# guzba/zippy

Hardware: NVIDIA H100
Metric: compress_level1_gzip_input_throughput (higher is better)
Workload: dtype u8

## Files before the change

zippy_b200/csrc/zb_deflate.cu:

```cuda
#include "zb_device.cuh"
#include "zb_kernels.h"
#include "zb_huff_warp.cuh"

#define LZ_THREADS (ZB_WARPS_PER_CHUNK * 32)
#define LZ_HASH_BITS 11
#define LZ_TABLE_ENTRIES (1 << LZ_HASH_BITS)
#define LZ_PRESEED 2048
#ifndef ZB_LZ1_RESOLVE_WINNER
#define ZB_LZ1_RESOLVE_WINNER 0
#endif
#define LZ_LANE_CAP 32

#define LZ_PIECE_BYTES ZB_REC_PIECE_BYTES
#define LZ_PHASES (ZB_SUB_BYTES / LZ_PIECE_BYTES)
#define LZ_PHASE_BYTES (ZB_CHUNK_BYTES / LZ_PHASES)
#define LZ_PHASE_HIST 1024
#define LZ_BATCH_LPW 2
#define LZ_BATCH_WINDOWS (32 / LZ_BATCH_LPW)
static_assert(LZ_PIECE_BYTES * ZB_WARPS_PER_CHUNK == LZ_PHASE_BYTES, "one piece per warp and phase");
static_assert(LZ_PIECE_BYTES / ZB_WINDOW % LZ_BATCH_WINDOWS == 0, "a batch of windows never straddles two pieces");

#define LZ_SM_DATA 0
#define LZ_SM_DATA_BYTES (LZ_PHASE_BYTES + LZ_PHASE_HIST + 64 + 384)
#define LZ_SM_TABLE (LZ_SM_DATA + LZ_SM_DATA_BYTES)
#define LZ_SM_TABLE_BYTES (ZB_WARPS_PER_CHUNK * LZ_TABLE_ENTRIES * 2)
#define LZ_SM_HIST (LZ_SM_TABLE + LZ_SM_TABLE_BYTES)
#define LZ_SM_HIST_BYTES (ZB_WARPS_PER_CHUNK * ZB_HIST_WORDS * 4)
#define LZ_SM_RING (LZ_SM_HIST + LZ_SM_HIST_BYTES)
#define LZ_SM_RING_BYTES (ZB_WARPS_PER_CHUNK * LZ_BATCH_WINDOWS * ZB_MATCH_SLOTS * 4)
#define LZ_SM_LMUL (LZ_SM_RING + LZ_SM_RING_BYTES)
#define LZ_LMUL_PIECE 33
#define LZ_LMUL_PQ 49
#define LZ_SM_LMUL_BYTES (56 * 4)
#define LZ_SM_PART (LZ_SM_LMUL + LZ_SM_LMUL_BYTES)
#define LZ_SM_PART_BYTES (ZB_WARPS_PER_CHUNK * 24)
#define LZ_SM_BAR (LZ_SM_PART + LZ_SM_PART_BYTES)
#define LZ_SM_TOTAL (LZ_SM_BAR + 16)
static_assert(LZ_TABLE_ENTRIES * 2 >= 4096, "a warp's table region must hold the CRC step table");
static_assert(3 * (LZ_SM_TOTAL + 1024) <= 233472, "three CTAs per SM");
static_assert(LZ_SM_PART % 8 == 0 && LZ_SM_TABLE % 16 == 0, "alignment");

__device__ __forceinline__ uint32_t lz_hash(uint32_t v) { return (v * 0x9E3779B1u) >> (32 - LZ_HASH_BITS); }
__device__ __forceinline__ uint32_t shl_clamp(uint32_t x, uint32_t n) {
  uint32_t r;
  asm("shl.b32 %0, %1, %2;" : "=r"(r) : "r"(x), "r"(n));
  return r;
}
__device__ __forceinline__ uint32_t low_mask(uint32_t n) { return shl_clamp(1u, n) - 1u; }

__device__ __forceinline__ uint32_t lz_final_rec(uint32_t mlen, uint32_t dist, int &lc, int &dc) {
  uint32_t le, de;
  lc = (int)zb_len_code_bf(mlen, le);
  dc = (int)zb_dist_code_bf(dist, de);
  return (uint32_t)lc | (le << 5) | ((uint32_t)dc << 10) | (de << 15);
}


__device__ __forceinline__ void lz_select(const uint8_t *data, uint32_t off0, uint32_t wb, uint32_t b1, uint32_t cur,
                                          uint32_t nvalid, uint32_t &m, uint32_t dist, uint32_t *ring_slot,
                                          uint32_t &sel, uint32_t &ism, uint32_t &endw) {
  const int lane = zb_lane();
  const uint32_t mm = __ballot_sync(ZB_FULL, m != 0);
  endw = 0;
  ism = 0;
  if (mm) {
    const uint32_t lbit = 1u << lane;
    const uint32_t endp = (uint32_t)lane + m;
    const uint32_t rest = shl_clamp(1u, endp) ? (mm >> endp) : 0u;
    uint32_t nc = rest ? endp + (uint32_t)(__ffs((int)rest) - 1) : 32u;
    uint32_t vis = 1u << (cur + (uint32_t)(__ffs((int)(mm >> cur)) - 1));
#pragma unroll
    for (int r = 0; r < 3; r++) {
      vis |= __reduce_or_sync(ZB_FULL, (vis & lbit) ? shl_clamp(1u, nc) : 0u);
      const uint32_t t = __shfl_sync(ZB_FULL, nc, (int)(nc & 31u));
      nc = nc < 32u ? t : 32u;
    }
    ism = vis;
    const int lastm = 31 - __clz((int)ism);
    const uint32_t cov = (ism & lbit) ? (low_mask(endp) & ~low_mask((uint32_t)lane)) : 0u;
    const uint32_t covered = __reduce_or_sync(ZB_FULL, cov);
    uint32_t mlast = __shfl_sync(ZB_FULL, m, lastm);
    if (mlast >= LZ_LANE_CAP) {
      const uint32_t md = __shfl_sync(ZB_FULL, dist, lastm);
      const uint32_t pos = wb + (uint32_t)lastm;
      const uint32_t off = off0 + pos + LZ_LANE_CAP + 8u * (uint32_t)lane;
      uint32_t x0 = zb_ld32_unaligned(data, off) ^ zb_ld32_unaligned(data, off - md);
      uint32_t x1 = zb_ld32_unaligned(data, off + 4) ^ zb_ld32_unaligned(data, off + 4 - md);
      uint32_t nm = x0 ? ((uint32_t)(__ffs((int)x0) - 1) >> 3) : 4u + (x1 ? ((uint32_t)(__ffs((int)x1) - 1) >> 3) : 4u);
      uint32_t stop = __ballot_sync(ZB_FULL, nm < 8u);
      if (stop) {
        int first = __ffs((int)stop) - 1;
        mlast = LZ_LANE_CAP + 8u * (uint32_t)first + __shfl_sync(ZB_FULL, nm, first);
      } else {
        mlast = LZ_LANE_CAP + 256u;
      }
      mlast = min(mlast, min((uint32_t)ZB_MAX_MATCH, b1 - pos));
      if (lane == lastm) m = mlast;
    }
    sel = ism | (~covered & ~low_mask(cur) & low_mask(nvalid));
    endw = (uint32_t)lastm + mlast;
    if (ism & lbit) {
      uint32_t rank = (uint32_t)__popc(ism & (lbit - 1u));
      ring_slot[rank] = (m - 3u) | ((dist - 1u) << 9);
    }
  } else {
    sel = low_mask(nvalid) & ~low_mask(cur);
  }
}

template <int LPW, bool LITS>
__device__ __forceinline__ void lz_batch_pass(const uint8_t *wdata, bool active, uint32_t ksel, uint32_t kism,
                                              const uint32_t *ring_win, uint32_t *whist, uint2 *gmask_w,
                                              uint32_t *grecs_piece, uint32_t &rec_base) {
  constexpr int NW = 32 / LPW;
  const uint32_t part = (uint32_t)zb_lane() / NW, wi = (uint32_t)zb_lane() % NW;
  if (active && part == 0) *gmask_w = make_uint2(ksel, kism);
  const uint32_t im = active ? kism : 0u;
  const uint32_t pm = (0xffffffffu >> (32 - 32 / LPW)) << (part * (32 / LPW));
  uint32_t s = (LITS && active) ? (ksel & ~kism & pm) : 0u;
  while (s) {
    const uint32_t bit = (uint32_t)(__ffs((int)s) - 1);
    s &= s - 1;
    const uint32_t sy = wdata[bit];
    atomicAdd(&whist[sy >> 1], 1u << ((sy & 1u) * 16u));
  }
  const uint32_t nmatch = (uint32_t)__popc(im);
  uint32_t incl = nmatch;
#pragma unroll
  for (int o = 1; o < NW; o <<= 1) {
    const uint32_t t = __shfl_up_sync(ZB_FULL, incl, o, NW);
    if (wi >= (uint32_t)o) incl += t;
  }
  uint32_t *grecs_w = grecs_piece + rec_base + incl - nmatch;
  rec_base += __shfl_sync(ZB_FULL, incl, NW - 1);
  for (uint32_t k = part; k < nmatch; k += LPW) {
    const uint32_t raw = ring_win[k];
    int lc, dc;
    const uint32_t fin = lz_final_rec((raw & 511u) + 3u, (raw >> 9) + 1u, lc, dc);
    grecs_w[k] = fin;
    const uint32_t s1 = 257u + (uint32_t)lc, s2 = (uint32_t)ZB_NUM_LITLEN + (uint32_t)dc;
    atomicAdd(&whist[s1 >> 1], 1u << ((s1 & 1u) * 16u));
    atomicAdd(&whist[s2 >> 1], 1u << ((s2 & 1u) * 16u));
  }
}

#ifndef ZB_LZ1_STAGE_CLOCKS
#define ZB_LZ1_STAGE_CLOCKS 0
#endif
enum { LZS_WAIT, LZS_CHECKSUM, LZS_SEED, LZS_PROBE, LZS_EXTEND, LZS_SELECT, LZS_BATCH, LZS_BARRIER, LZS_N };
#if ZB_LZ1_STAGE_CLOCKS
__device__ unsigned long long zb_lz1_stage_clk[LZS_N];
#define LZ_CLK_DECL                          \
  unsigned long long clk_acc[LZS_N] = {};    \
  long long clk_t = clock64();
#define LZ_CLK(s)                            \
  if (MODE == 1) {                           \
    const long long clk_n = clock64();       \
    clk_acc[s] += (unsigned long long)(clk_n - clk_t); \
    clk_t = clk_n;                           \
  }
#define LZ_CLK_PUBLISH()                                                                           \
  if (MODE == 1 && lane == 0) {                                                                    \
    _Pragma("unroll") for (int s_ = 0; s_ < LZS_N; s_++) atomicAdd(&zb_lz1_stage_clk[s_], clk_acc[s_]); \
  }
extern "C" int zb200_lz1_stage_clocks(unsigned long long *out) {
  unsigned long long zero[LZS_N] = {};
  if (cudaMemcpyFromSymbol(out, zb_lz1_stage_clk, sizeof(zero)) != cudaSuccess) return -1;
  return cudaMemcpyToSymbol(zb_lz1_stage_clk, zero, sizeof(zero)) == cudaSuccess ? 0 : -1;
}
#else
#define LZ_CLK_DECL
#define LZ_CLK(s)
#define LZ_CLK_PUBLISH()
#endif

template <int MODE, int CK>
__global__ void __launch_bounds__(LZ_THREADS, 3)
    k_lz(const uint8_t *__restrict__ src, const ZbChunkDesc *__restrict__ desc, uint2 *__restrict__ masks,
         uint32_t *__restrict__ recs, uint16_t *__restrict__ hist, ZbChunkCheck *__restrict__ chk,
         const ZbCrcTables *__restrict__ tabs, uint32_t max_dist) {
  extern __shared__ __align__(128) uint8_t smem[];
  uint8_t *data = smem + LZ_SM_DATA;
  uint16_t *table_all = reinterpret_cast<uint16_t *>(smem + LZ_SM_TABLE);
  uint32_t *hist_all = reinterpret_cast<uint32_t *>(smem + LZ_SM_HIST);
  uint32_t *ring_all = reinterpret_cast<uint32_t *>(smem + LZ_SM_RING);
  uint32_t *lane_mul = reinterpret_cast<uint32_t *>(smem + LZ_SM_LMUL);
  uint64_t *part = reinterpret_cast<uint64_t *>(smem + LZ_SM_PART);
  uint64_t *bar = reinterpret_cast<uint64_t *>(smem + LZ_SM_BAR);

  const uint32_t chunk = blockIdx.x;
  const ZbChunkDesc d = desc[chunk];
  const uint32_t len = d.len;
  const int tid = (int)threadIdx.x, lane = tid & 31;
  const int warp = (int)__reduce_max_sync(ZB_FULL, (uint32_t)tid >> 5);

  if (tid == 0) {
    zb_mbar_init(bar, 1);
    zb_fence_mbar_init();
  }
  __syncthreads();
  const uint32_t mis = (uint32_t)((uintptr_t)(src + d.src_off) & 15u);

  uint16_t *table = table_all + warp * LZ_TABLE_ENTRIES;
  uint32_t *ring = ring_all + warp * LZ_BATCH_WINDOWS * ZB_MATCH_SLOTS;
  uint2 *gmask = masks + (size_t)chunk * ZB_WINDOWS_PER_CHUNK;
  uint32_t acc_crc = 0;
  uint64_t acc_a = 0, acc_b = 0;
  LZ_CLK_DECL

  for (uint32_t ph = 0; ph < LZ_PHASES; ph++) {
    const uint32_t pbase = ph * LZ_PHASE_BYTES;
    if (ph && pbase >= len) break;
    const uint32_t sbase = ph ? pbase - LZ_PHASE_HIST : 0u;
    if (ph) __syncthreads();
    LZ_CLK(LZS_BARRIER)
    if (tid == 0 && len) {
      zb_fence_proxy_async();
      zb_stage_chunk(data, src + d.src_off + sbase, min(len, pbase + LZ_PHASE_BYTES + 384u) - sbase, bar);
    }
    if (CK & ZB_CK_CRC) {
      uint32_t *crc_tab = reinterpret_cast<uint32_t *>(table);
      for (int i = lane; i < 1024; i += 32) crc_tab[i] = (&tabs->mul1024[0][0])[i];
    }
    if (ph == 0) {
      for (int i = tid; i < ZB_WARPS_PER_CHUNK * ZB_HIST_WORDS; i += LZ_THREADS) hist_all[i] = 0;
      if (tid < 33) lane_mul[tid] = tabs->lane_mul[tid];
      if (tid >= 64 && tid < 80) lane_mul[LZ_LMUL_PIECE + tid - 64] = tabs->piece_mul[tid - 64];
      if (tid >= 96 && tid < 100) lane_mul[LZ_LMUL_PQ + tid - 96] = tabs->pq_mul[tid - 96];
      __syncthreads();
    } else {
      __syncwarp();
    }
    if (len) zb_mbar_wait(bar, ph & 1u);
    LZ_CLK(LZS_WAIT)

    const uint32_t b0 = pbase + (uint32_t)warp * LZ_PIECE_BYTES;
    if (b0 >= len) continue;
    const uint32_t b1 = min(b0 + LZ_PIECE_BYTES, len);
    const uint32_t doff = mis - sbase;
    uint32_t *whist = hist_all + (b0 / ZB_SUB_BYTES) * ZB_HIST_WORDS;

    if (CK) {
      ZbCheck c = zb_warp_checksums<LZ_PIECE_BYTES, LZ_LMUL_PQ, CK>(data, doff + b0, b1 - b0,
                                                                    reinterpret_cast<const uint32_t *>(table), lane_mul);
      const uint32_t after = len - b1;
      if (after) {
        if (CK & ZB_CK_CRC) {
          const uint32_t shift = ((after & (LZ_PIECE_BYTES - 1)) == 0) ? lane_mul[LZ_LMUL_PIECE + after / LZ_PIECE_BYTES]
                                                                       : zb_xpow8_t(tabs->pow2, after);
          c.crc_raw = zb_gf2_mul(c.crc_raw, shift);
        }
        if (CK & ZB_CK_ADLER) c.b_sum += (uint64_t)after * c.a_sum;
      }
      acc_crc ^= c.crc_raw;
      acc_a += c.a_sum;
      acc_b += c.b_sum;
      __syncwarp();
    }
    LZ_CLK(LZS_CHECKSUM)

    if (MODE == 1) {
      uint4 ff = make_uint4(~0u, ~0u, ~0u, ~0u);
      uint4 *t4 = reinterpret_cast<uint4 *>(table);
      for (int i = lane; i < LZ_TABLE_ENTRIES * 2 / 16; i += 32) t4[i] = ff;
      __syncwarp();
      for (uint32_t s = b0 - min((uint32_t)LZ_PRESEED, b0 - sbase); s < b0; s += 32) {
        const uint32_t p = s + (uint32_t)lane;
        const bool can = p + 4 <= len;
        const uint32_t h = lz_hash(zb_ld32_unaligned(data, doff + p));
        if (can) table[h] = (uint16_t)p;
#if ZB_LZ1_RESOLVE_WINNER
        __syncwarp();
        for (;;) {
          const bool lost = can && table[h] < (uint16_t)p;
          if (!__any_sync(ZB_FULL, lost)) break;
          if (lost) table[h] = (uint16_t)p;
          __syncwarp();
        }
#endif
      }
      __syncwarp();
    }
    LZ_CLK(LZS_SEED)
    uint32_t entry = b0;
    uint32_t ksel = 0, kism = 0;
    uint32_t *grecs = recs + (size_t)chunk * ZB_RECS_PER_CHUNK + (b0 >> 2);
    uint32_t rec_base = 0;
    const uint32_t bl = (uint32_t)lane & (LZ_BATCH_WINDOWS - 1u);
    for (uint32_t wb = b0; wb < b1; wb += 32) {
      const uint32_t win = wb >> 5, slot = win & (LZ_BATCH_WINDOWS - 1u);
      uint32_t sel = 0, ism = 0;
      if (entry < wb + 32) {
        const uint32_t p = wb + (uint32_t)lane;
        const uint32_t nvalid = min(32u, b1 - wb);
        const uint32_t cur = entry - wb;
        uint32_t m = 0, c = 0, lit = 0;
        if (MODE == 2) {
          const uint32_t x = doff + p;
          lit = data[x];
          const uint32_t eq0 = __ballot_sync(ZB_FULL, p != 0u && lit == data[x - 1u]);
          const uint32_t eq1 = __ballot_sync(ZB_FULL, data[x + 32u] == data[x + 31u]);
          const uint32_t ahead = __funnelshift_r(eq0, eq1, (uint32_t)lane);
          const uint32_t run = ahead == ~0u ? (uint32_t)LZ_LANE_CAP : (uint32_t)(__ffs((int)~ahead) - 1);
          const uint32_t limit = p < b1 ? b1 - p : 0u;
          const uint32_t r = run < (uint32_t)LZ_LANE_CAP ? min(run, limit) : run;
          if (p >= entry && r >= 3u && limit >= 3u) m = r;
          c = p - 1u;
        }
        if (MODE == 1) {
          const uint32_t *wp = reinterpret_cast<const uint32_t *>(data) + ((doff + p) >> 2);
          const uint32_t sp = ((doff + p) & 3u) * 8u;
          const uint32_t p0 = wp[0], p1 = wp[1];
          const uint32_t v = __funnelshift_r(p0, p1, sp);
          lit = v & 255u;
          const bool can = (p + 4 <= len);
          const uint32_t h = lz_hash(v);
          c = table[h];
          __syncwarp();
          if (can) table[h] = (uint16_t)p;
#if ZB_LZ1_RESOLVE_WINNER
          __syncwarp();
          for (;;) {
            const bool lost = can && table[h] < (uint16_t)p;
            if (!__any_sync(ZB_FULL, lost)) break;
            if (lost) table[h] = (uint16_t)p;
            __syncwarp();
          }
#endif
          LZ_CLK(LZS_PROBE)
          const uint32_t limit = p < b1 ? min((uint32_t)ZB_MAX_MATCH, b1 - p) : 0u;
          if (can && c < p && p - c <= max_dist && p >= entry && limit >= ZB_MIN_MATCH) {
            const uint32_t *wc = reinterpret_cast<const uint32_t *>(data) + ((doff + c) >> 2);
            const uint32_t sc = ((doff + c) & 3u) * 8u;
            uint32_t hp = p1, hc = wc[1];
            uint32_t np = wp[2], nq = wc[2], np2 = wp[3], nq2 = wc[3];
            if (__funnelshift_r(wc[0], hc, sc) == v) {
              m = 4;
#pragma unroll 1
              for (int k = 2;; k += 2) {
                const uint32_t x = __funnelshift_r(hp, np, sp) ^ __funnelshift_r(hc, nq, sc);
                const uint32_t x2 = __funnelshift_r(np, np2, sp) ^ __funnelshift_r(nq, nq2, sc);
                if (x) {
                  m += (uint32_t)(__ffs((int)x) - 1) >> 3;
                  break;
                }
                if (k == LZ_LANE_CAP / 4) {
                  m += 4;
                  break;
                }
                if (x2) {
                  m += 4u + ((uint32_t)(__ffs((int)x2) - 1) >> 3);
                  break;
                }
                m += 8;
                hp = np2;
                hc = nq2;
                np = wp[k + 2];
                nq = wc[k + 2];
                np2 = wp[k + 3];
                nq2 = wc[k + 3];
              }
              if (m < LZ_LANE_CAP) m = min(m, limit);
            }
          }
          LZ_CLK(LZS_EXTEND)
        }
        uint32_t endw;
        lz_select(data, doff, wb, b1, cur, nvalid, m, p - c, ring + slot * ZB_MATCH_SLOTS, sel, ism, endw);
        entry = wb + max(endw, nvalid);
        if (MODE != 0 && ((sel & ~ism) >> lane & 1u)) atomicAdd(&whist[lit >> 1], 1u << ((lit & 1u) * 16u));
        LZ_CLK(LZS_SELECT)
      }
      if (bl == slot) {
        ksel = sel;
        kism = ism;
      }
      if (slot == LZ_BATCH_WINDOWS - 1u || wb + 32 >= b1) {
        __syncwarp();
        const uint32_t bwin = win - slot + bl;
        lz_batch_pass<LZ_BATCH_LPW, MODE == 0>(data + (uint32_t)(doff + (bwin << 5)), bl <= slot, ksel, kism, ring + bl * ZB_MATCH_SLOTS,
                                    whist, gmask + bwin, grecs, rec_base);
        ksel = kism = 0;
        __syncwarp();
      }
      LZ_CLK(LZS_BATCH)
    }
  }
  if (lane == 0) {
    part[warp * 3 + 0] = acc_crc;
    part[warp * 3 + 1] = acc_a;
    part[warp * 3 + 2] = acc_b;
  }
  __syncthreads();
  {
    uint32_t *gh = reinterpret_cast<uint32_t *>(hist + (size_t)chunk * ZB_WARPS_PER_CHUNK * ZB_HIST_SYMS);
    for (int i = tid; i < ZB_WARPS_PER_CHUNK * ZB_HIST_WORDS; i += LZ_THREADS) gh[i] = hist_all[i];
  }
  LZ_CLK(LZS_BARRIER)
  LZ_CLK_PUBLISH()
  if (tid == 0) {
    uint32_t raw = 0;
    uint64_t a = 0, b = 0;
    for (int w = 0; w < ZB_WARPS_PER_CHUNK; w++) {
      raw ^= (uint32_t)part[w * 3 + 0];
      a += part[w * 3 + 1];
      b += part[w * 3 + 2];
    }
    ZbChunkCheck cc;
    cc.crc_raw = raw;
    cc.adler = (CK & ZB_CK_ADLER) ? zb_adler_from_sums(a % ZB_ADLER_MOD, b % ZB_ADLER_MOD, len) : 0u;
    chk[chunk] = cc;
  }
}

#define LZ2_HIST 32768
#define LZ2_SEG_BYTES ZB_SUB_BYTES
#define LZ2_SEGS ((ZB_CHUNK_BYTES + LZ2_HIST) / LZ2_SEG_BYTES)
#define LZ2_BUCKET_BITS 11
#define LZ2_BUCKETS (1 << LZ2_BUCKET_BITS)
#define LZ2_TABLES_PER_CTA (ZB_WARPS_PER_CHUNK + LZ2_SEGS)
#define LZ2_RING_WINDOWS 8
#define LZ2_SM_DATA_BYTES (ZB_CHUNK_BYTES + LZ2_HIST + 64 + 384)
#define LZ2_SM_HIST (LZ2_SM_DATA_BYTES)
#define LZ2_SM_RING (LZ2_SM_HIST + LZ_SM_HIST_BYTES)
#define LZ2_SM_RING_BYTES (ZB_WARPS_PER_CHUNK * LZ2_RING_WINDOWS * ZB_MATCH_SLOTS * 4)
#define LZ2_SM_CRC (LZ2_SM_RING + LZ2_SM_RING_BYTES)
#define LZ2_SM_LMUL (LZ2_SM_CRC + 4096)
#define LZ2_SM_PART (LZ2_SM_LMUL + LZ_SM_LMUL_BYTES)
#define LZ2_SM_LIST (LZ2_SM_PART + LZ_SM_PART_BYTES)
#define LZ2_SM_BAR (LZ2_SM_LIST + 8 * LZ_THREADS * 2)
#define LZ2_SM_TOTAL (LZ2_SM_BAR + 16)
static_assert(2 * (LZ2_SM_TOTAL + 1024) <= 233472, "two CTAs per SM");

#ifndef LZ2_CTAS_PER_SM
#define LZ2_CTAS_PER_SM 1
#endif
#ifndef LZ2_STATIC_BITS
#define LZ2_STATIC_BITS 13
#endif
__device__ __forceinline__ uint32_t lz2_hash_mul(uint32_t v) { return v * 0x9E3779B1u; }
__device__ __forceinline__ uint32_t lz2_hash(uint32_t v) { return lz2_hash_mul(v) >> (32 - LZ2_BUCKET_BITS); }

__device__ __forceinline__ uint2 lz2_push(uint2 b, uint32_t e) {
  uint2 r;
  r.y = __funnelshift_l(b.x, b.y, 16);
  r.x = (b.x << 16) | (e & 0xffffu);
  return r;
}

__device__ __forceinline__ void lz2_clear_table(uint2 *tab, int bytes = LZ2_BUCKETS * 8) {
  const uint4 ff = make_uint4(~0u, ~0u, ~0u, ~0u);
  uint4 *t4 = reinterpret_cast<uint4 *>(tab);
  for (int i = zb_lane(); i < bytes / 16; i += 32) __stcg(&t4[i], ff);
}

__device__ __forceinline__ uint2 lz2_probe_insert(uint2 *tab, uint32_t h, bool can, uint32_t qwin, uint32_t &grp) {
  const int lane = zb_lane();
  grp = __match_any_sync(ZB_FULL, can ? h : (0x80000000u | (uint32_t)lane));
  uint2 old = make_uint2(~0u, ~0u);
  if (can) old = __ldcg(&tab[h]);
  __syncwarp();
  if (can && lane == 31 - __clz((int)grp)) {
    uint2 nb = old;
    for (uint32_t g = grp; g; g &= g - 1) nb = lz2_push(nb, qwin + (uint32_t)(__ffs((int)g) - 1));
    __stcg(&tab[h], nb);
  }
  __syncwarp();
  return old;
}

struct Lz2Pos {
  const uint32_t *data32;
  uint32_t poff;
  uint32_t q;
  uint32_t v;
  uint32_t lim;
  uint32_t limit, stop;
};

#define LZ2_LIST 8
__device__ __forceinline__ void lz2_verify(const Lz2Pos &P, uint32_t e, bool search, uint16_t *dl, uint32_t &n) {
  const uint32_t d = (P.q - e) & 0xffffu;
  if (!search || (d - 1u) >= P.lim) return;
  const uint32_t co = P.poff - d;
  const uint32_t *wc = P.data32 + (co >> 2);
  if (__funnelshift_r(wc[0], wc[1], (co & 3u) * 8u) != P.v) return;
  if (n < LZ2_LIST) dl[n * (uint32_t)LZ_THREADS] = (uint16_t)d;
  n += n < LZ2_LIST ? 1u : 0u;
}
__device__ __forceinline__ void lz2_extend(const Lz2Pos &P, const uint8_t *data, uint32_t d, uint32_t good, uint32_t &m,
                                           uint32_t &dist, int &budget) {
  const uint32_t co = P.poff - d;
  budget--;
  if (m >= 4 && data[co + m] != data[P.poff + m]) {
    if (m >= good && budget > 1) budget = 1;
    return;
  }
  const uint32_t *wc = P.data32 + (co >> 2);
  const uint32_t sc = (co & 3u) * 8u;
  const uint32_t *wp = P.data32 + (P.poff >> 2);
  const uint32_t sp = (P.poff & 3u) * 8u;
  uint32_t hp = wp[1], hc = wc[1];
  uint32_t mc = 4;
#pragma unroll 1
  for (int j = 2; j <= LZ_LANE_CAP / 4; j++) {
    const uint32_t np = wp[j], nq = wc[j];
    const uint32_t x = __funnelshift_r(hp, np, sp) ^ __funnelshift_r(hc, nq, sc);
    if (x) {
      mc += (uint32_t)(__ffs((int)x) - 1) >> 3;
      break;
    }
    mc += 4;
    hp = np;
    hc = nq;
  }
  mc = min(mc, P.limit);
  if (mc > m) {
    m = mc;
    dist = d;
  }
  if (m >= good && budget > 1) budget = 1;
}

__device__ __forceinline__ void stage_dict_chunk(uint8_t *data, const uint8_t *chunk, uint32_t len, uint32_t hb,
                                                 const uint8_t *wend, uint64_t *bar) {
  const uint32_t cmis = (uint32_t)((uintptr_t)chunk & 15u);
  const uint32_t mis = (cmis - hb) & 15u, a0 = hb + mis - cmis;
  const uint32_t cbytes = (cmis + len + 15u) & ~15u;
  zb_mbar_expect_tx(bar, a0 + cbytes);
  for (uint32_t done = 0; done < a0;) {
    const uint32_t n = min(a0 - done, 32768u);
    zb_tma_load_1d(data + done, wend - hb - mis + done, n, bar);
    done += n;
  }
  for (uint32_t done = 0; done < cbytes;) {
    const uint32_t n = min(cbytes - done, 32768u);
    zb_tma_load_1d(data + a0 + done, chunk - cmis + done, n, bar);
    done += n;
  }
}
__device__ __forceinline__ void fix_dict_head(uint8_t *data, const uint8_t *chunk, uint32_t hb, const uint8_t *wend) {
  const uint32_t cmis = (uint32_t)((uintptr_t)chunk & 15u);
  const uint32_t mis = (cmis - hb) & 15u;
  const uint32_t q = hb - min(hb, cmis) + threadIdx.x;
  if (q < hb) {
    data[mis + q] = wend[(int)q - (int)hb];
    zb_fence_proxy_async();
  }
}

template <bool DICT, int MINM = ZB_MIN_MATCH>
__global__ void __launch_bounds__(LZ_THREADS, 2)
    k_lz2(const uint8_t *__restrict__ src, const ZbChunkDesc *__restrict__ desc, uint2 *__restrict__ masks,
          uint32_t *__restrict__ recs, uint16_t *__restrict__ hist, ZbChunkCheck *__restrict__ chk,
          const ZbCrcTables *__restrict__ tabs, uint2 *__restrict__ tables, uint32_t n_chunks, ZbLz2Params prm,
          const ZbMemberDict *__restrict__ mdict) {
  extern __shared__ __align__(128) uint8_t smem[];
  uint8_t *data = smem;
  uint32_t *hist_all = reinterpret_cast<uint32_t *>(smem + LZ2_SM_HIST);
  uint32_t *ring_all = reinterpret_cast<uint32_t *>(smem + LZ2_SM_RING);
  uint32_t *crc_tab = reinterpret_cast<uint32_t *>(smem + LZ2_SM_CRC);
  uint32_t *lane_mul = reinterpret_cast<uint32_t *>(smem + LZ2_SM_LMUL);
  uint64_t *part = reinterpret_cast<uint64_t *>(smem + LZ2_SM_PART);
  uint64_t *bar = reinterpret_cast<uint64_t *>(smem + LZ2_SM_BAR);
  const int tid = (int)threadIdx.x, lane = tid & 31, warp = tid >> 5;
  uint16_t *dlist = reinterpret_cast<uint16_t *>(smem + LZ2_SM_LIST) + tid;
  uint32_t *whist = hist_all + warp * ZB_HIST_WORDS;
  uint32_t *ring = ring_all + warp * LZ2_RING_WINDOWS * ZB_MATCH_SLOTS;
  uint2 *cta_tabs = tables + (size_t)blockIdx.x * LZ2_TABLES_PER_CTA * LZ2_BUCKETS;
  uint2 *own = cta_tabs + (size_t)warp * LZ2_BUCKETS;
  uint2 *stat = cta_tabs + (size_t)ZB_WARPS_PER_CHUNK * LZ2_BUCKETS;

  if (tid == 0) {
    zb_mbar_init(bar, 1);
    zb_fence_mbar_init();
  }
  for (int i = tid; i < 1024; i += LZ_THREADS) crc_tab[i] = (&tabs->mul1024[0][0])[i];
  if (tid < 33) lane_mul[tid] = tabs->lane_mul[tid];
  if (tid >= 64 && tid < 72) lane_mul[33 + tid - 64] = tabs->sub_mul[tid - 64];
  if (tid >= 96 && tid < 100) lane_mul[41 + tid - 96] = tabs->quart_mul[tid - 96];
  __syncthreads();

  uint32_t phase = 0;
  for (uint32_t chunk = blockIdx.x; chunk < n_chunks; chunk += gridDim.x) {
    const ZbChunkDesc d = desc[chunk];
    const uint32_t len = d.len, hb = d.pad;
    const uint32_t hg = (0u - hb) & (LZ2_SEG_BYTES - 1u);
    const uint8_t *rsrc = src + d.src_off - hb;
    const uint32_t mis = (uint32_t)((uintptr_t)rsrc & 15u);
    const uint32_t off0 = mis + hb;
    const uint32_t rlen = hb + len;
    const uint8_t *wend = DICT && (d.flags & ZB_CHUNK_DICT) ? mdict[d.member].wend : nullptr;
    if (DICT && wend) {
      if (tid == 0) stage_dict_chunk(data, src + d.src_off, len, hb, wend, bar);
    } else if (tid == 0 && rlen) {
      zb_stage_chunk(data, rsrc, rlen, bar);
    }
    for (int i = tid; i < ZB_WARPS_PER_CHUNK * ZB_HIST_WORDS; i += LZ_THREADS) hist_all[i] = 0;
    lz2_clear_table(own);
    __syncthreads();
    if (rlen) {
      zb_mbar_wait(bar, phase);
      phase ^= 1u;
    }
    if (DICT && wend) {
      fix_dict_head(data, src + d.src_off, hb, wend);
      __syncthreads();
    }

    const uint32_t b0 = (uint32_t)warp * ZB_SUB_BYTES;
    const uint32_t b1 = min(b0 + ZB_SUB_BYTES, len);
    {
      ZbCheck c;
      c.crc_raw = 0;
      c.a_sum = c.b_sum = 0;
      uint32_t n = b0 < len ? b1 - b0 : 0;
      if (n) {
        c = zb_warp_checksums(data, off0 + b0, n, crc_tab, lane_mul);
        const uint32_t after = len - b1;
        if (after) {
          const uint32_t shift = ((after & (ZB_SUB_BYTES - 1)) == 0) ? lane_mul[33 + after / ZB_SUB_BYTES] : zb_xpow8_t(tabs->pow2, after);
          c.crc_raw = zb_gf2_mul(c.crc_raw, shift);
          c.b_sum += (uint64_t)after * c.a_sum;
        }
      }
      if (lane == 0) {
        part[warp * 3 + 0] = c.crc_raw;
        part[warp * 3 + 1] = c.a_sum;
        part[warp * 3 + 2] = c.b_sum;
      }
      __syncwarp();
    }

    {
      const uint32_t nseg = (hg + rlen + LZ2_SEG_BYTES - 1) / LZ2_SEG_BYTES;
      const uint32_t seg0 = (hg + hb) / LZ2_SEG_BYTES, sg0 = seg0 > prm.hist_segs ? seg0 - prm.hist_segs : 0u;
      for (uint32_t sg = sg0 + (uint32_t)warp; sg + 1 < nseg; sg += ZB_WARPS_PER_CHUNK) {
        uint2 *tab = stat + (size_t)sg * LZ2_BUCKETS;
        lz2_clear_table(tab, (1 << LZ2_STATIC_BITS) * 2);
        __syncwarp();
        uint16_t *tab16 = reinterpret_cast<uint16_t *>(tab);
        const uint32_t q0 = sg ? sg * LZ2_SEG_BYTES - hg : 0u, q1 = (sg + 1) * LZ2_SEG_BYTES - hg;
        for (uint32_t s = q0; s < q1; s += 32) {
          const uint32_t q = s + (uint32_t)lane;
          const uint32_t v = zb_ld32_unaligned(data, mis + q);
          const uint32_t hs = lz2_hash_mul(v) >> (32 - LZ2_STATIC_BITS);
          const bool can = q + 4 <= rlen && q < q1;
          const uint32_t grp = __match_any_sync(ZB_FULL, can ? hs : (0x80000000u | (uint32_t)lane));
          if (can && lane == 31 - __clz((int)grp)) __stcg(&tab16[hs], (uint16_t)q);
        }
        __syncwarp();
      }
    }
    __syncthreads();

    if (b0 < len) {
      const uint32_t myseg = (hg + hb + b0) / LZ2_SEG_BYTES;
      uint32_t entry = b0;
      uint32_t ksel = 0, kism = 0;
      uint2 *gmask = masks + (size_t)chunk * ZB_WINDOWS_PER_CHUNK;
      uint32_t *grecs = recs + (size_t)chunk * ZB_RECS_PER_CHUNK;
      uint32_t rec_base = 0;
      for (uint32_t wb = b0; wb < b1; wb += 32) {
        const uint32_t win = wb >> 5, slot = win & (LZ2_RING_WINDOWS - 1u);
        if ((wb & (ZB_REC_PIECE_BYTES - 1u)) == 0u) rec_base = 0;
        const uint32_t p = wb + (uint32_t)lane;
        const uint32_t q = hb + p;
// ... 706 lines not shown
```

Measured before the change: 80.77.

## Process two LZ windows per iteration with early hash probing of the second

In level-1 mode, the match loop now handles two consecutive 32-byte windows in one iteration when both fit inside the current batch. It loads and hashes both windows and does the hash-table probe and insert for the second window up front, so those memory latencies overlap with the first window's match extension and selection. If the first window's selected match covers the whole second window, the speculative table insert is rolled back by restoring the old candidate. The match-extension loop is factored into a helper, which adds register pressure and extra branch paths in exchange for more memory-level parallelism.

```diff
diff --git a/zippy_b200/csrc/zb_deflate.cu b/zippy_b200/csrc/zb_deflate.cu
--- a/zippy_b200/csrc/zb_deflate.cu
+++ b/zippy_b200/csrc/zb_deflate.cu
@@ -108,6 +108,42 @@
   }
 }
 
+__device__ __forceinline__ uint32_t lz1_extend(const uint32_t *wp, uint32_t sp, uint32_t v, uint32_t p1,
+                                               const uint32_t *wc, uint32_t sc, uint32_t limit) {
+  uint32_t m = 0;
+  uint32_t hp = p1, hc = wc[1];
+  uint32_t np = wp[2], nq = wc[2], np2 = wp[3], nq2 = wc[3];
+  if (__funnelshift_r(wc[0], hc, sc) == v) {
+    m = 4;
+#pragma unroll 1
+    for (int k = 2;; k += 2) {
+      const uint32_t x = __funnelshift_r(hp, np, sp) ^ __funnelshift_r(hc, nq, sc);
+      const uint32_t x2 = __funnelshift_r(np, np2, sp) ^ __funnelshift_r(nq, nq2, sc);
+      if (x) {
+        m += (uint32_t)(__ffs((int)x) - 1) >> 3;
+        break;
+      }
+      if (k == LZ_LANE_CAP / 4) {
+        m += 4;
+        break;
+      }
+      if (x2) {
+        m += 4u + ((uint32_t)(__ffs((int)x2) - 1) >> 3);
+        break;
+      }
+      m += 8;
+      hp = np2;
+      hc = nq2;
+      np = wp[k + 2];
+      nq = wc[k + 2];
+      np2 = wp[k + 3];
+      nq2 = wc[k + 3];
+    }
+    if (m < LZ_LANE_CAP) m = min(m, limit);
+  }
+  return m;
+}
+
 template <int LPW, bool LITS>
 __device__ __forceinline__ void lz_batch_pass(const uint8_t *wdata, bool active, uint32_t ksel, uint32_t kism,
                                               const uint32_t *ring_win, uint32_t *whist, uint2 *gmask_w,
@@ -288,9 +324,75 @@
     uint32_t rec_base = 0;
     const uint32_t bl = (uint32_t)lane & (LZ_BATCH_WINDOWS - 1u);
     for (uint32_t wb = b0; wb < b1; wb += 32) {
-      const uint32_t win = wb >> 5, slot = win & (LZ_BATCH_WINDOWS - 1u);
+      uint32_t win = wb >> 5, slot = win & (LZ_BATCH_WINDOWS - 1u);
       uint32_t sel = 0, ism = 0;
-      if (entry < wb + 32) {
+      if (MODE == 1 && entry < wb + 32 && slot != LZ_BATCH_WINDOWS - 1u && wb + 64 <= b1) {
+        const uint32_t pA = wb + (uint32_t)lane, pB = pA + 32u;
+        const uint32_t *wa = reinterpret_cast<const uint32_t *>(data) + ((doff + pA) >> 2), *wq = wa + 8;
+        const uint32_t sp = ((doff + pA) & 3u) * 8u;
+        const uint32_t a1 = wa[1], q1 = wq[1];
+        const uint32_t vA = __funnelshift_r(wa[0], a1, sp), vB = __funnelshift_r(wq[0], q1, sp);
+        const bool canA = pA + 4 <= len, canB = pB + 4 <= len;
+        const uint32_t hA = lz_hash(vA), hB = lz_hash(vB);
+        const uint32_t cA = table[hA];
+        __syncwarp();
+        if (canA) table[hA] = (uint16_t)pA;
+#if ZB_LZ1_RESOLVE_WINNER
+        __syncwarp();
+        for (;;) {
+          const bool lost = canA && table[hA] < (uint16_t)pA;
+          if (!__any_sync(ZB_FULL, lost)) break;
+          if (lost) table[hA] = (uint16_t)pA;
+          __syncwarp();
+        }
+#endif
+        __syncwarp();
+        const uint32_t cB = table[hB];
+        __syncwarp();
+        if (canB) table[hB] = (uint16_t)pB;
+#if ZB_LZ1_RESOLVE_WINNER
+        __syncwarp();
+        for (;;) {
+          const bool lost = canB && table[hB] < (uint16_t)pB;
+          if (!__any_sync(ZB_FULL, lost)) break;
+          if (lost) table[hB] = (uint16_t)pB;
+          __syncwarp();
+        }
+#endif
+        LZ_CLK(LZS_PROBE)
+        uint32_t m = 0, endw;
+        if (canA && cA < pA && pA - cA <= max_dist && pA >= entry)
+          m = lz1_extend(wa, sp, vA, a1, reinterpret_cast<const uint32_t *>(data) + ((doff + cA) >> 2),
+                         ((doff + cA) & 3u) * 8u, min((uint32_t)ZB_MAX_MATCH, b1 - pA));
+        LZ_CLK(LZS_EXTEND)
+        lz_select(data, doff, wb, b1, entry - wb, 32u, m, pA - cA, ring + slot * ZB_MATCH_SLOTS, sel, ism, endw);
+        entry = wb + max(endw, 32u);
+        if ((sel & ~ism) >> lane & 1u) atomicAdd(&whist[(vA & 255u) >> 1], 1u << ((vA & 1u) * 16u));
+        LZ_CLK(LZS_SELECT)
+        if (bl == slot) {
+          ksel = sel;
+          kism = ism;
+        }
+        wb += 32;
+        win++;
+        slot++;
+        if (entry < wb + 32) {
+          const uint32_t limit = min((uint32_t)ZB_MAX_MATCH, b1 - pB);
+          m = 0;
+          if (canB && cB < pB && pB - cB <= max_dist && pB >= entry && limit >= ZB_MIN_MATCH)
+            m = lz1_extend(wq, sp, vB, q1, reinterpret_cast<const uint32_t *>(data) + ((doff + cB) >> 2),
+                           ((doff + cB) & 3u) * 8u, limit);
+          LZ_CLK(LZS_EXTEND)
+          lz_select(data, doff, wb, b1, entry - wb, 32u, m, pB - cB, ring + slot * ZB_MATCH_SLOTS, sel, ism, endw);
+          entry = wb + max(endw, 32u);
+          if ((sel & ~ism) >> lane & 1u) atomicAdd(&whist[(vB & 255u) >> 1], 1u << ((vB & 1u) * 16u));
+          LZ_CLK(LZS_SELECT)
+        } else {
+          if (canB) table[hB] = (uint16_t)cB;
+          __syncwarp();
+          sel = ism = 0;
+        }
+      } else if (entry < wb + 32) {
         const uint32_t p = wb + (uint32_t)lane;
         const uint32_t nvalid = min(32u, b1 - wb);
         const uint32_t cur = entry - wb;
@@ -329,40 +431,9 @@
 #endif
           LZ_CLK(LZS_PROBE)
           const uint32_t limit = p < b1 ? min((uint32_t)ZB_MAX_MATCH, b1 - p) : 0u;
-          if (can && c < p && p - c <= max_dist && p >= entry && limit >= ZB_MIN_MATCH) {
-            const uint32_t *wc = reinterpret_cast<const uint32_t *>(data) + ((doff + c) >> 2);
-            const uint32_t sc = ((doff + c) & 3u) * 8u;
-            uint32_t hp = p1, hc = wc[1];
-            uint32_t np = wp[2], nq = wc[2], np2 = wp[3], nq2 = wc[3];
-            if (__funnelshift_r(wc[0], hc, sc) == v) {
-              m = 4;
-#pragma unroll 1
-              for (int k = 2;; k += 2) {
-                const uint32_t x = __funnelshift_r(hp, np, sp) ^ __funnelshift_r(hc, nq, sc);
-                const uint32_t x2 = __funnelshift_r(np, np2, sp) ^ __funnelshift_r(nq, nq2, sc);
-                if (x) {
-                  m += (uint32_t)(__ffs((int)x) - 1) >> 3;
-                  break;
-                }
-                if (k == LZ_LANE_CAP / 4) {
-                  m += 4;
-                  break;
-                }
-                if (x2) {
-                  m += 4u + ((uint32_t)(__ffs((int)x2) - 1) >> 3);
-                  break;
-                }
-                m += 8;
-                hp = np2;
-                hc = nq2;
-                np = wp[k + 2];
-                nq = wc[k + 2];
-                np2 = wp[k + 3];
-                nq2 = wc[k + 3];
-              }
-              if (m < LZ_LANE_CAP) m = min(m, limit);
-            }
-          }
+          if (can && c < p && p - c <= max_dist && p >= entry && limit >= ZB_MIN_MATCH)
+            m = lz1_extend(wp, sp, v, p1, reinterpret_cast<const uint32_t *>(data) + ((doff + c) >> 2),
+                           ((doff + c) & 3u) * 8u, limit);
           LZ_CLK(LZS_EXTEND)
         }
         uint32_t endw;
```

Result: no change. 80.88 (median of 6 runs) (+0.1%).
